# YuanchenBei/ColdRec

Measured on AMD Instinct MI355X. Metric: ranked items/sec (full-catalogue eval), higher is better.
Workload: dtype f32; 1 GPU; configs[3] full-catalogue eval: 1000000-row user table x 10000000 items, d=128, k=20, f32 tables, user block 131072 per step, rated CSR (mean ~50) + 20% cold-item bitmap ('warm' setting), item table row-sharded over 1 GPU(s); items=10000000, dim=128, k=20, parallelism=single GPU

## Files before the change

coldrec_amd/csrc/score_screen.hip:

```cpp
#include <math.h>

#include "score_topk_common.h"

#include <hipcub/device/device_radix_sort.hpp>

namespace crh_score {
namespace {

constexpr int SD = 128;
constexpr int FB_SCRATCH_SLICES = 64;

__device__ __forceinline__ float up_float(double x) {
    if (!(x <= 3.0e38)) return __builtin_inff();
    float f = (float)x;
    if ((double)f < x) f = __uint_as_float(__float_as_uint(f) + 1u);
    return f;
}

__device__ __forceinline__ int scale_exp(const unsigned* stats, int word) {
    const float m = __uint_as_float(stats[word]);
    if (!(m > 0.0f) || !(m <= 3.4e38f)) return 0;
    int E;
    frexpf(m, &E);
    return 15 - E;
}

__device__ __forceinline__ _Float16 to_f16(float x, int e) {
    const float y = ldexpf(x, e);
    _Float16 hv = (_Float16)y;
    if (fabsf((float)hv) < 6.103515625e-05f) hv = (_Float16)0.0f;
    return hv;
}

__device__ __forceinline__ float wave_max(float v) {
#pragma unroll
    for (int o = 32; o >= 1; o >>= 1) v = fmaxf(v, __shfl_xor(v, o));
    return v;
}

constexpr unsigned SCREEN_KEY_NONFINITE = 0x7F80u;
template <bool KEYS>
__global__ __launch_bounds__(256) void screen_maxabs_kernel(const float* __restrict__ tab, const int32_t* __restrict__ rows,
                                                            int64_t n_rows, unsigned* __restrict__ stats, int word,
                                                            uint16_t* __restrict__ keys) {
    const int64_t n4 = n_rows * (SD / 4);
    float m = 0.0f;
    for (int64_t e = (int64_t)blockIdx.x * 256 + threadIdx.x; e < n4; e += (int64_t)gridDim.x * 256) {
        const int64_t r = e / (SD / 4);
        const int64_t row = rows ? (int64_t)rows[r] : r;
        const f32x4 x = *reinterpret_cast<const f32x4*>(tab + row * SD + 4 * (e % (SD / 4)));
#pragma unroll
        for (int c = 0; c < 4; ++c) {
            const float ax = fabsf(x[c]);
            if (ax <= 3.4028235e38f) m = fmaxf(m, ax);
        }
        if constexpr (KEYS) {
            float ss = x[0] * x[0] + x[1] * x[1] + x[2] * x[2] + x[3] * x[3];
#pragma unroll
            for (int o = 16; o >= 1; o >>= 1) ss += __shfl_xor(ss, o);
            if ((threadIdx.x & 31) == 0)
                keys[r] = (uint16_t)(ss <= 3.4028235e38f ? __float_as_uint(ss) >> 16 : SCREEN_KEY_NONFINITE);
        }
    }
    __shared__ float red[4];
    m = wave_max(m);
    if ((threadIdx.x & 63) == 0) red[threadIdx.x >> 6] = m;
    __syncthreads();
    if (threadIdx.x == 0) {
        const float b = fmaxf(fmaxf(red[0], red[1]), fmaxf(red[2], red[3]));
        if (b > 0.0f) atomicMax(stats + word, __float_as_uint(b));
    }
}

__device__ __forceinline__ void row_sums(const f32x4& x0, const f32x4& x1, _Float16 (&hv)[8], int e, double& sxx, double& sdd,
                                         double& shh) {
    const double inv = ldexp(1.0, -e);
    sxx = 0.0; sdd = 0.0; shh = 0.0;
#pragma unroll
    for (int c = 0; c < 8; ++c) {
        const float x = c < 4 ? x0[c & 3] : x1[c & 3];
        hv[c] = to_f16(x, e);
        const double xh = (double)(float)hv[c] * inv;
        const double dx = (double)x - xh;
        sxx += (double)x * (double)x;
        sdd += dx * dx;
        shh += xh * xh;
    }
#pragma unroll
    for (int o = 1; o < 16; o <<= 1) {
        sxx += __shfl_xor(sxx, o);
        sdd += __shfl_xor(sdd, o);
        shh += __shfl_xor(shh, o);
    }
}

__device__ __forceinline__ float up_norm(double s) { return up_float(sqrt(s) * (1.0 + 0x1p-30)); }

constexpr int LIVE_WPB = 256;

__device__ __forceinline__ unsigned live_word(const uint32_t* __restrict__ bitmap, int64_t w, int64_t g0, int64_t g1) {
    const int64_t w0 = g0 >> 5, n_words = ((g1 - 1) >> 5) - w0 + 1;
    if (w >= n_words) return 0u;
    unsigned m = ~bitmap[w0 + w];
    const int64_t lo = (w0 + w) << 5;
    if (lo < g0) m &= ~0u << (int)(g0 - lo);
    if (lo + 32 > g1) m &= ~0u >> (int)(lo + 32 - g1);
    return m;
}

__device__ __forceinline__ unsigned block_excl_sum(unsigned v, unsigned* total) {
    __shared__ unsigned wsum[4];
    const int lane = threadIdx.x & 63, wv = threadIdx.x >> 6;
    unsigned inc = v;
#pragma unroll
    for (int o = 1; o < 64; o <<= 1) {
        const unsigned t = __shfl_up(inc, o);
        if (lane >= o) inc += t;
    }
    if (lane == 63) wsum[wv] = inc;
    __syncthreads();
    unsigned before = 0;
    for (int q = 0; q < wv; ++q) before += wsum[q];
    *total = wsum[0] + wsum[1] + wsum[2] + wsum[3];
    return before + inc - v;
}

__global__ __launch_bounds__(256) void screen_live_count_kernel(const uint32_t* __restrict__ bitmap, int64_t g0, int64_t g1,
                                                                unsigned* __restrict__ blocksum) {
    const unsigned c = __popc(live_word(bitmap, (int64_t)blockIdx.x * LIVE_WPB + threadIdx.x, g0, g1));
    unsigned total;
    block_excl_sum(c, &total);
    if (threadIdx.x == 0) blocksum[blockIdx.x] = total;
}

__global__ __launch_bounds__(256) void screen_live_scan_kernel(unsigned* __restrict__ blocksum, int64_t n_blocks,
                                                               unsigned* __restrict__ n_live) {
    const int64_t per = (n_blocks + 255) / 256;
    const int64_t lo = threadIdx.x * per < n_blocks ? threadIdx.x * per : n_blocks, hi = lo + per < n_blocks ? lo + per : n_blocks;
    unsigned sum = 0;
    for (int64_t q = lo; q < hi; ++q) sum += blocksum[q];
    unsigned total;
    unsigned run = block_excl_sum(sum, &total);
    for (int64_t q = lo; q < hi; ++q) {
        const unsigned c = blocksum[q];
        blocksum[q] = run;
        run += c;
    }
    if (threadIdx.x == 0) *n_live = total;
}

__global__ __launch_bounds__(256) void screen_idmap_kernel(const uint32_t* __restrict__ bitmap, int64_t g0, int64_t g1,
                                                           const unsigned* __restrict__ blocksum, int32_t* __restrict__ idmap) {
    const int64_t w = (int64_t)blockIdx.x * LIVE_WPB + threadIdx.x;
    unsigned m = live_word(bitmap, w, g0, g1);
    unsigned total;
    int64_t pos = (int64_t)blocksum[blockIdx.x] + block_excl_sum(__popc(m), &total);
    const int id0 = (int)(((g0 >> 5) + w) << 5);
    while (m) {
        idmap[pos++] = id0 + __builtin_ctz(m);
        m &= m - 1;
    }
}

__global__ __launch_bounds__(256) void screen_sortkey_kernel(const int32_t* __restrict__ idmap, const uint16_t* __restrict__ rowkeys,
                                                             const unsigned* __restrict__ n_live, int64_t item_base, int64_t n_slots,
                                                             uint16_t* __restrict__ skeys) {
    const int64_t q = (int64_t)blockIdx.x * 256 + threadIdx.x;
    if (q >= n_slots) return;
    skeys[q] = q < (int64_t)*n_live ? (uint16_t)~rowkeys[(int64_t)idmap[q] - item_base] : (uint16_t)0xFFFFu;
}

__global__ __launch_bounds__(256) void screen_mapkeys_kernel(const uint16_t* __restrict__ skeys, int64_t n, int32_t* __restrict__ out) {
    const int64_t q = (int64_t)blockIdx.x * 256 + threadIdx.x;
    if (q < n) out[q] = (int32_t)(uint16_t)~skeys[q];
}

__global__ __launch_bounds__(256) void screen_items_kernel(const float* __restrict__ v, int64_t n_items, const uint32_t* __restrict__ bitmap,
                                                           int64_t item_base, _Float16* __restrict__ packed, unsigned* __restrict__ stats,
                                                           int64_t prefix, const int32_t* __restrict__ idmap) {
    const int e = scale_exp(stats, 0);
    const int64_t TP = prefix >> 5, n_live = idmap ? (int64_t)stats[SCREEN_STAT_LIVE] : 0;
    const int64_t T = idmap ? TP + ((n_live + 31) >> 5) : (n_items + 31) >> 5;
    float mr = 0.0f, mn = 0.0f, mh = 0.0f;
    u32x4* dst = reinterpret_cast<u32x4*>(packed);
    for (int64_t t = blockIdx.x; t < T; t += gridDim.x) {
        for (int p = 0; p < 2; ++p) {
            const int u = threadIdx.x + 256 * p, r = u >> 4, c = u & 15;
            int64_t row = (t << 5) + r;
            bool masked;
            if (idmap != nullptr && t >= TP) {
                const int64_t q = row - prefix;
                masked = q >= n_live;
                row = (int64_t)idmap[masked ? n_live - 1 : q] - item_base;
            } else {
                if (row >= n_items) row = n_items - 1;
                masked = bitmap != nullptr && ((bitmap[(item_base + row) >> 5] >> ((item_base + row) & 31)) & 1u);
            }
            const float* src = v + row * SD + 8 * c;
            const f32x4 x0 = *reinterpret_cast<const f32x4*>(src), x1 = *reinterpret_cast<const f32x4*>(src + 4);
            _Float16 hv[8];
            double sxx, sdd, shh;
            row_sums(x0, x1, hv, e, sxx, sdd, shh);
            u32x4 o = u32x4{0u, 0u, 0u, 0u};
            if (!masked) {
                o = __builtin_bit_cast(u32x4, f16x8{hv[0], hv[1], hv[2], hv[3], hv[4], hv[5], hv[6], hv[7]});
                mr = fmaxf(mr, up_norm(sdd));
                mn = fmaxf(mn, up_norm(sxx));
                mh = fmaxf(mh, up_norm(shh));
                if (sdd != sdd || sxx != sxx) mr = __builtin_inff();
            }
            dst[(t * 8 + (c >> 1)) * 64 + (c & 1) * 32 + r] = o;
        }
    }
    __shared__ float red[3][4];
    mr = wave_max(mr);
    mn = wave_max(mn);
    mh = wave_max(mh);
    if ((threadIdx.x & 63) == 0) {
        red[0][threadIdx.x >> 6] = mr;
        red[1][threadIdx.x >> 6] = mn;
        red[2][threadIdx.x >> 6] = mh;
    }
    __syncthreads();
    if (threadIdx.x < 3) {
        const float b = fmaxf(fmaxf(red[threadIdx.x][0], red[threadIdx.x][1]), fmaxf(red[threadIdx.x][2], red[threadIdx.x][3]));
        if (b > 0.0f) atomicMax(stats + 2 + threadIdx.x, __float_as_uint(b));
    }
}

__global__ __launch_bounds__(256) void screen_users_kernel(const float* __restrict__ uemb, const int32_t* __restrict__ users,
                                                           int64_t n_users, _Float16* __restrict__ uh, float* __restrict__ ustat,
                                                           const unsigned* __restrict__ stats) {
    const int e = scale_exp(stats, 1);
    const int64_t n_units = n_users * 16;
    for (int64_t w = (int64_t)blockIdx.x * 256 + threadIdx.x; w < ((n_units + 255) & ~(int64_t)255); w += (int64_t)gridDim.x * 256) {
        const int64_t j = (w < n_units ? w : n_units - 1) >> 4;
        const int c = (int)(w & 15);
        const int64_t row = users ? (int64_t)users[j] : j;
        const float* src = uemb + row * SD + 8 * c;
        const f32x4 x0 = *reinterpret_cast<const f32x4*>(src), x1 = *reinterpret_cast<const f32x4*>(src + 4);
        _Float16 hv[8];
        double sxx, sdd, shh;
        row_sums(x0, x1, hv, e, sxx, sdd, shh);
        if (w < n_units) {
            reinterpret_cast<u32x4*>(uh)[j * 16 + c] = __builtin_bit_cast(u32x4, f16x8{hv[0], hv[1], hv[2], hv[3], hv[4], hv[5], hv[6], hv[7]});
            if (c == 0) {
                const bool bad = sxx != sxx || sdd != sdd;
                ustat[3 * j + 0] = bad ? __builtin_inff() : up_norm(sxx);
                ustat[3 * j + 1] = bad ? __builtin_inff() : up_norm(shh);
                ustat[3 * j + 2] = bad ? __builtin_inff() : up_norm(sdd);
            }
        }
    }
}

__device__ __forceinline__ float exact_chain(const float* __restrict__ u, const float* __restrict__ v) {
    float s = 0.0f;
#pragma unroll 8
    for (int q = 0; q < SD; q += 4) {
        const f32x4 a = *reinterpret_cast<const f32x4*>(u + q), b = *reinterpret_cast<const f32x4*>(v + q);
        s = __builtin_fmaf(a.x, b.x, s);
        s = __builtin_fmaf(a.y, b.y, s);
        s = __builtin_fmaf(a.z, b.z, s);
        s = __builtin_fmaf(a.w, b.w, s);
    }
    return s;
}

__device__ __forceinline__ bool lane_in_list(const int32_t* __restrict__ col, int64_t lo, int64_t hi, int gi) {
    while (lo < hi) {
        const int64_t mid = lo + ((hi - lo) >> 1);
        const int x = col[mid];
        if (x == gi) return true;
        if (x < gi) lo = mid + 1;
        else hi = mid;
    }
    return false;
}

__global__ __launch_bounds__(256) void screen_certify_kernel(ScreenArgs s) {
    const int lane = threadIdx.x & 63;
    const int64_t slot = (int64_t)blockIdx.x * 4 + (threadIdx.x >> 6);
    if (slot >= s.n_users) return;
    const int KP = s.kp, K = s.k;
    const bool mine = lane < KP;
    int gi = CRH_PAD_IDX;
    float a = CRH_NEG_INF;
    if (mine) {
        gi = s.cand_idx[slot * KP + lane];
        a = s.cand_score[slot * KP + lane];
    }
    const bool real = mine && gi != CRH_PAD_IDX && (int64_t)gi >= s.item_base && (int64_t)gi < s.item_base + s.n_items;
    bool masked = false;
    if (real && s.bitmap) masked = (s.bitmap[gi >> 5] >> (gi & 31)) & 1u;
    if (real && !masked && s.rated_rowptr) masked = lane_in_list(s.rated_col, s.rated_rowptr[slot], s.rated_rowptr[slot + 1], gi);
    const int64_t urow = s.users ? (int64_t)s.users[slot] : slot;
    float sc = CRH_NEG_INF;
    if (real) sc = exact_chain(s.user_emb + urow * SD, s.item_emb + ((int64_t)gi - s.item_base) * SD);
    const bool ok = !mine || (real && !masked && __builtin_isfinite(a) && __builtin_isfinite(sc));
    int rank = 0;
    for (int j = 0; j < KP; ++j) {
        const float sj = __shfl(sc, j);
        const int ij = __shfl(gi, j);
        rank += (j != lane && crh_better(sj, ij, sc, gi)) ? 1 : 0;
    }
    const unsigned long long kth = __ballot(mine && rank == K - 1);
    const float ek = __shfl(sc, kth ? __builtin_ctzll(kth) : 0);
    const float a_last = __shfl(a, KP - 1);
    bool cert = s.mode != 3 && __ballot(!ok) == 0ull && kth != 0ull;
    if (cert) {
        const float* us = s.ustat + 3 * slot;
        const float R = __uint_as_float(s.stats[2]), N = __uint_as_float(s.stats[3]), Nh = __uint_as_float(s.stats[4]);
        const double gd = SD * 0x1p-24 / (1.0 - SD * 0x1p-24), gp = 0x1p-12;
        double B = (double)us[0] * R + (double)us[2] * Nh + gd * (double)us[0] * N + gp * (double)us[1] * Nh + 0x1p-126;
        B *= 1.0 + 0x1p-20;
        const double A = (double)a_last * ldexp(1.0, -(scale_exp(s.stats, 0) + scale_exp(s.stats, 1)));
        double thr = A + B;
        thr += fabs(thr) * 0x1p-50;
        cert = (double)ek > thr && ek > CRH_MASKED_SCORE;
    }
    if (cert) {
        if (mine && rank < K) {
            s.out_score[slot * K + rank] = sc;
            s.out_idx[slot * K + rank] = gi;
        }
    } else if (lane == 0) {
        const unsigned f = atomicAdd(s.stats + 5, 1u);
        s.fail_list[f] = (int32_t)slot;
    }
}

constexpr int64_t FB_WAVES = 2048 * 4;
constexpr int64_t FB_MIN_ITEMS = 1024;
constexpr int FB_FANIN = 64;
constexpr int FB_SLICES_MAX = FB_FANIN * FB_FANIN;
__device__ __forceinline__ int fb_slices(const ScreenArgs& s, int64_t count) {
    if (count <= 0) return 1;
    int64_t S = (FB_WAVES + count - 1) / count;
    const int64_t by_items = (s.n_items + FB_MIN_ITEMS - 1) / FB_MIN_ITEMS;
    const int64_t by_scratch = s.n_users * s.n_slices / count;
    if (S > by_items) S = by_items;
    if (S > by_scratch) S = by_scratch;
    if (S > FB_SLICES_MAX) S = FB_SLICES_MAX;
    return S < 1 ? 1 : (int)S;
}

__global__ __launch_bounds__(256) void screen_fallback_kernel(ScreenArgs s) {
    __shared__ float ush[4][SD];
    __shared__ float lsh[4][32];
    __shared__ int lih[4][32];
    __shared__ int cnth[4];
    const int lane = threadIdx.x & 63, wv = threadIdx.x >> 6;
    const int K = s.k;
    const int64_t count = s.stats[5];
    const int S = fb_slices(s, count);
    const int64_t n_work = count * S;
    float* ls = lsh[wv];
    int* li = lih[wv];
    int* cnt = &cnth[wv];
    for (int64_t w = (int64_t)blockIdx.x * 4 + wv; w < n_work; w += (int64_t)gridDim.x * 4) {
        const int64_t f = w / S;
        const int z = (int)(w % S);
        const int64_t slot = s.fail_list[f];
        const int64_t urow = s.users ? (int64_t)s.users[slot] : slot;
        ush[wv][lane] = s.user_emb[urow * SD + lane];
        ush[wv][lane + 64] = s.user_emb[urow * SD + lane + 64];
        if (lane == 0) *cnt = 0;
        const int64_t lo = s.n_items * z / S, hi = s.n_items * (z + 1) / S;
        float tau = CRH_NEG_INF;
        for (int64_t base = lo; base < hi; base += 64) {
            const int64_t i = base + lane;
            const bool valid = i < hi;
            const int gl = (int)(s.item_base + (valid ? i : lo));
            const bool bm = valid && s.bitmap && ((s.bitmap[gl >> 5] >> (gl & 31)) & 1u);
            float raw = CRH_NEG_INF;
            if (valid) {
                if (bm) {
                    raw = 0.0f;
#pragma unroll 8
                    for (int q = 0; q < SD; ++q) raw = __builtin_fmaf(ush[wv][q], 0.0f, raw);
                } else {
                    raw = exact_chain(ush[wv], s.item_emb + i * SD);
                }
            }
            unsigned long long cand = __ballot(valid && raw > tau);
            const unsigned long long bms = __ballot(bm);
            while (cand) {
                const int L = __builtin_ctzll(cand);
                cand &= cand - 1;
                float sc = __shfl(raw, L);
                const int g = (int)(s.item_base + base + L);
                const int n = __builtin_amdgcn_readfirstlane(*cnt);
                if (wave_list_rejects(ls, li, n, K, sc, g)) continue;
                bool masked = (bms >> L) & 1ull;
                if (!masked && s.rated_rowptr) masked = wave_is_masked(g, slot, s.rated_rowptr, s.rated_col, nullptr, lane);
                if (masked) sc = CRH_MASKED_SCORE;
                wave_list_insert(ls, li, cnt, K, sc, g, lane);
                tau = wave_list_tau(ls, __builtin_amdgcn_readfirstlane(*cnt), K);
            }
        }
        const int n = __builtin_amdgcn_readfirstlane(*cnt);
        const int64_t o = (f * S + z) * K;
        wave_list_store(ls, li, n, K, s.part_score + o, s.part_idx + o, lane);
    }
}

__global__ __launch_bounds__(256) void screen_fallback_merge_kernel(ScreenArgs s, int level) {
    __shared__ float lsh[4][32];
    __shared__ int lih[4][32];
    __shared__ int cnth[4];
    const int lane = threadIdx.x & 63, wv = threadIdx.x >> 6;
    const int K = s.k;
    const int64_t count = s.stats[5];
    const int S = fb_slices(s, count);
    const int last = S <= FB_FANIN ? 0 : 1;
    if (level > last) return;
    const int stride = level == 0 ? 1 : FB_FANIN;
    const int span = stride * FB_FANIN;
    const int G = (S + span - 1) / span;
    float* ls = lsh[wv];
    int* li = lih[wv];
    int* cnt = &cnth[wv];
    for (int64_t w = (int64_t)blockIdx.x * 4 + wv; w < count * G; w += (int64_t)gridDim.x * 4) {
        const int64_t f = w / G;
        const int z0 = (int)(w % G) * span;
        if (lane == 0) *cnt = 0;
        for (int z = z0; z < z0 + span && z < S; z += stride) {
            const int64_t o = (f * S + z) * K;
            const float es = lane < K ? s.part_score[o + lane] : CRH_NEG_INF;
            const int ei = lane < K ? s.part_idx[o + lane] : CRH_PAD_IDX;
            unsigned long long m = __ballot(lane < K && ei != CRH_PAD_IDX);
            while (m) {
                const int L = __builtin_ctzll(m);
                m &= m - 1;
                const float sc = __shfl(es, L);
                const int g = __shfl(ei, L);
                const int n = __builtin_amdgcn_readfirstlane(*cnt);
                if (n >= K && !crh_better(sc, g, ls[K - 1], li[K - 1])) break;
                wave_list_insert(ls, li, cnt, K, sc, g, lane);
            }
        }
        const int n = __builtin_amdgcn_readfirstlane(*cnt);
        if (level == last) {
            const int64_t slot = s.fail_list[f];
            wave_list_store(ls, li, n, K, s.out_score + slot * K, s.out_idx + slot * K, lane);
        } else {
            const int64_t o = (f * S + z0) * K;
            wave_list_store(ls, li, n, K, s.part_score + o, s.part_idx + o, lane);
        }
    }
}

}

int screen_fallback_slices(int64_t n_items) {
    const int64_t s = n_items / 4096;
    return (int)(s < 1 ? 1 : (s > FB_SCRATCH_SLICES ? FB_SCRATCH_SLICES : s));
}

size_t screen_scan_bytes(int64_t n_main) { return (size_t)((n_main + 31) / 32 / LIVE_WPB + 2) * sizeof(unsigned); }

int64_t screen_map_slots(int64_t n_main) { return ((n_main + 31) / 32 + 1) * 32; }

size_t screen_sort_bytes(int64_t n_slots) { return (size_t)n_slots * 8 + ((size_t)1 << 20); }

int launch_screen_map(const uint32_t* bitmap, int64_t item_base, int64_t n_items, int64_t prefix, unsigned* n_live, unsigned* scan,
                      int32_t* idmap, const ScreenOrder* ord, hipStream_t st) {
    const int64_t g0 = item_base + prefix, g1 = item_base + n_items;
    const int64_t n_words = ((g1 - 1) >> 5) - (g0 >> 5) + 1, nb = (n_words + LIVE_WPB - 1) / LIVE_WPB;
    hipLaunchKernelGGL(screen_live_count_kernel, dim3((unsigned)nb), dim3(256), 0, st, bitmap, g0, g1, scan);
    CRH_HIP(hipGetLastError());
    hipLaunchKernelGGL(screen_live_scan_kernel, dim3(1), dim3(256), 0, st, scan, nb, n_live);
    CRH_HIP(hipGetLastError());
    hipLaunchKernelGGL(screen_idmap_kernel, dim3((unsigned)nb), dim3(256), 0, st, bitmap, g0, g1, scan, idmap);
    CRH_HIP(hipGetLastError());
    if (ord == nullptr) return CRH_OK;
    const int64_t n_slots = screen_map_slots(n_items - prefix);
    hipLaunchKernelGGL(screen_sortkey_kernel, dim3((unsigned)((n_slots + 255) / 256)), dim3(256), 0, st, idmap, ord->rowkeys, n_live,
                       item_base, n_slots, ord->skeys_in);
    CRH_HIP(hipGetLastError());
    size_t need = 0;
    CRH_HIP(hipcub::DeviceRadixSort::SortPairs(nullptr, need, ord->skeys_in, ord->skeys_out, idmap, ord->idmap, (int)n_slots, 0, 16, st));
    if (need > ord->sort_tmp_bytes) {
        crh_set_error("screened route: the ordered map's sort asks for %zu bytes of temporary storage, %zu are reserved", need,
                      ord->sort_tmp_bytes);
        return CRH_ERR_WS;
    }
    need = ord->sort_tmp_bytes;
    CRH_HIP(hipcub::DeviceRadixSort::SortPairs(ord->sort_tmp, need, ord->skeys_in, ord->skeys_out, idmap, ord->idmap, (int)n_slots, 0, 16, st));
    return CRH_OK;
}

int launch_screen_prep_items(const ScreenArgs& s, unsigned* stats, _Float16* packed, int64_t prefix, int32_t* idmap, unsigned* scan,
                             const ScreenOrder* ord, hipStream_t st) {
    const int64_t T = (s.n_items + 31) / 32;
    if (ord != nullptr)
        hipLaunchKernelGGL(screen_maxabs_kernel<true>, dim3(2048), dim3(256), 0, st, s.item_emb, nullptr, s.n_items, stats, 0, ord->rowkeys);
    else
        hipLaunchKernelGGL(screen_maxabs_kernel<false>, dim3(2048), dim3(256), 0, st, s.item_emb, nullptr, s.n_items, stats, 0, nullptr);
    CRH_HIP(hipGetLastError());
    if (idmap != nullptr) {
        const int rc = launch_screen_map(s.bitmap, s.item_base, s.n_items, prefix, stats + SCREEN_STAT_LIVE, scan, idmap, ord, st);
        if (rc != CRH_OK) return rc;
        if (ord != nullptr) idmap = ord->idmap;
    }
    hipLaunchKernelGGL(screen_items_kernel, dim3((unsigned)(T < 4096 ? T : 4096)), dim3(256), 0, st, s.item_emb, s.n_items, s.bitmap,
                       s.item_base, packed, stats, prefix, idmap);
    CRH_HIP(hipGetLastError());
    return CRH_OK;
}

int launch_screen_prep_users(const ScreenArgs& s, _Float16* uh, hipStream_t st) {
    hipLaunchKernelGGL(screen_maxabs_kernel<false>, dim3(256), dim3(256), 0, st, s.user_emb, s.users, s.n_users, s.stats, 1, nullptr);
    CRH_HIP(hipGetLastError());
    const int64_t ub = (s.n_users * 16 + 255) / 256;
    hipLaunchKernelGGL(screen_users_kernel, dim3((unsigned)(ub < 2048 ? ub : 2048)), dim3(256), 0, st, s.user_emb, s.users, s.n_users,
                       uh, s.ustat, s.stats);
    CRH_HIP(hipGetLastError());
    return CRH_OK;
}

int screen_map_only(const uint32_t* bitmap, const float* item_emb, int64_t n_items, int64_t item_base, int64_t prefix, int ordered,
                    int32_t* map_out, int32_t* keys_out, int64_t* count, hipStream_t st) {
    auto al = [](size_t x) { return (x + 255) & ~(size_t)255; };
    const int64_t n_main = n_items - prefix, n_slots = screen_map_slots(n_main);
    const size_t o_scan = 256, o_map = o_scan + al(screen_scan_bytes(n_main)), o_rk = o_map + al((size_t)n_slots * 4),
                 o_k0 = o_rk + al((size_t)n_items * 2), o_k1 = o_k0 + al((size_t)n_slots * 2), o_m1 = o_k1 + al((size_t)n_slots * 2),
                 o_tmp = o_m1 + al((size_t)n_slots * 4), total = o_tmp + screen_sort_bytes(n_slots);
    char* buf = nullptr;
    CRH_HIP(hipMalloc(reinterpret_cast<void**>(&buf), total));
    ScreenOrder ord;
    ord.rowkeys = reinterpret_cast<uint16_t*>(buf + o_rk);
    ord.skeys_in = reinterpret_cast<uint16_t*>(buf + o_k0);
    ord.skeys_out = reinterpret_cast<uint16_t*>(buf + o_k1);
    ord.idmap = reinterpret_cast<int32_t*>(buf + o_m1);
    ord.sort_tmp = buf + o_tmp;
    ord.sort_tmp_bytes = screen_sort_bytes(n_slots);
    unsigned* stats = reinterpret_cast<unsigned*>(buf);
    int32_t* idmap = reinterpret_cast<int32_t*>(buf + o_map);
    int rc = CRH_OK;
    unsigned live = 0;
    hipError_t e = hipMemsetAsync(buf, 0, 256, st);
    if (e == hipSuccess) {
        hipLaunchKernelGGL(screen_maxabs_kernel<true>, dim3(2048), dim3(256), 0, st, item_emb, nullptr, n_items, stats, 0, ord.rowkeys);
        e = hipGetLastError();
    }
    if (e == hipSuccess) rc = launch_screen_map(bitmap, item_base, n_items, prefix, stats + SCREEN_STAT_LIVE, reinterpret_cast<unsigned*>(buf + o_scan), idmap, &ord, st);
    if (e == hipSuccess && rc == CRH_OK) {
        hipLaunchKernelGGL(screen_mapkeys_kernel, dim3((unsigned)((n_main + 255) / 256)), dim3(256), 0, st,
                           ordered ? ord.skeys_out : ord.skeys_in, n_main, keys_out);
        e = hipGetLastError();
    }
    if (e == hipSuccess && rc == CRH_OK)
        e = hipMemcpyAsync(map_out, ordered ? ord.idmap : idmap, (size_t)n_main * 4, hipMemcpyDeviceToDevice, st);
    if (e == hipSuccess && rc == CRH_OK) e = hipMemcpyAsync(&live, stats + SCREEN_STAT_LIVE, 4, hipMemcpyDeviceToHost, st);
    if (e == hipSuccess) e = hipStreamSynchronize(st);
    (void)hipFree(buf);
    CRH_HIP(e);
    if (rc == CRH_OK) *count = (int64_t)live;
    return rc;
}

int launch_screen_certify(const ScreenArgs& s, hipStream_t st) {
    hipLaunchKernelGGL(screen_certify_kernel, dim3((unsigned)((s.n_users + 3) / 4)), dim3(256), 0, st, s);
    CRH_HIP(hipGetLastError());
    hipLaunchKernelGGL(screen_fallback_kernel, dim3((unsigned)(FB_WAVES / 4)), dim3(256), 0, st, s);
    CRH_HIP(hipGetLastError());
    for (int level = 0; level < 2; ++level) {
        hipLaunchKernelGGL(screen_fallback_merge_kernel, dim3(512), dim3(256), 0, st, s, level);
        CRH_HIP(hipGetLastError());
    }
    return CRH_OK;
}

}
```

Measured before the change: 6721 billion items/s.

## Batch fallback users per wave and seed fallback threshold from screen candidates

Result: no change. 6761 billion items/s, median of 6 (+0.6%).

```diff
diff --git a/coldrec_amd/csrc/score_screen.hip b/coldrec_amd/csrc/score_screen.hip
--- a/coldrec_amd/csrc/score_screen.hip
+++ b/coldrec_amd/csrc/score_screen.hip
@@ -324,11 +324,32 @@
             s.out_score[slot * K + rank] = sc;
             s.out_idx[slot * K + rank] = gi;
         }
-    } else if (lane == 0) {
-        const unsigned f = atomicAdd(s.stats + 5, 1u);
-        s.fail_list[f] = (int32_t)slot;
-    }
-}
+    } else {
+        const bool good = real && !masked && __builtin_isfinite(sc);
+        const float s2 = good ? sc : CRH_NEG_INF;
+        const int g2 = good ? gi : CRH_PAD_IDX;
+        int r2 = 0;
+        for (int j = 0; j < KP; ++j) {
+            const float sj = __shfl(s2, j);
+            const int ij = __shfl(g2, j);
+            r2 += (j != lane && crh_better(sj, ij, s2, g2)) ? 1 : 0;
+        }
+        const unsigned long long k2 = __ballot(good && r2 == K - 1);
+        float seed = __shfl(s2, k2 ? __builtin_ctzll(k2) : 0);
+        if (k2 == 0ull || !(seed > CRH_MASKED_SCORE)) seed = CRH_NEG_INF;
+        if (lane == 0) {
+            const unsigned f = atomicAdd(s.stats + 5, 1u);
+            s.fail_list[f] = (int32_t)slot;
+            s.ustat[3 * slot] = seed;
+        }
+    }
+}
+
+#ifdef CRH_SCREEN_FALLBACK_PER_USER
+constexpr int FB_GROUP = 1;
+#else
+constexpr int FB_GROUP = 4;
+#endif
 
 constexpr int64_t FB_WAVES = 2048 * 4;
 constexpr int64_t FB_MIN_ITEMS = 1024;
@@ -336,7 +357,8 @@
 constexpr int FB_SLICES_MAX = FB_FANIN * FB_FANIN;
 __device__ __forceinline__ int fb_slices(const ScreenArgs& s, int64_t count) {
     if (count <= 0) return 1;
-    int64_t S = (FB_WAVES + count - 1) / count;
+    const int64_t groups = (count + FB_GROUP - 1) / FB_GROUP;
+    int64_t S = (FB_WAVES + groups - 1) / groups;
     const int64_t by_items = (s.n_items + FB_MIN_ITEMS - 1) / FB_MIN_ITEMS;
     const int64_t by_scratch = s.n_users * s.n_slices / count;
     if (S > by_items) S = by_items;
@@ -345,63 +367,108 @@
     return S < 1 ? 1 : (int)S;
 }
 
+template <int NU>
+__device__ __forceinline__ void exact_chain_group(const float* __restrict__ u, const float* __restrict__ v, float (&sc)[FB_GROUP]) {
+#pragma unroll
+    for (int j = 0; j < NU; ++j) sc[j] = 0.0f;
+#pragma unroll 8
+    for (int q = 0; q < SD; q += 4) {
+        const f32x4 b = *reinterpret_cast<const f32x4*>(v + q);
+#pragma unroll
+        for (int j = 0; j < NU; ++j) {
+            const f32x4 a = *reinterpret_cast<const f32x4*>(u + j * SD + q);
+            sc[j] = __builtin_fmaf(a.x, b.x, sc[j]);
+            sc[j] = __builtin_fmaf(a.y, b.y, sc[j]);
+            sc[j] = __builtin_fmaf(a.z, b.z, sc[j]);
+            sc[j] = __builtin_fmaf(a.w, b.w, sc[j]);
+        }
+    }
+}
+
 __global__ __launch_bounds__(256) void screen_fallback_kernel(ScreenArgs s) {
-    __shared__ float ush[4][SD];
-    __shared__ float lsh[4][32];
-    __shared__ int lih[4][32];
-    __shared__ int cnth[4];
+    __shared__ __attribute__((aligned(16))) float ush[4][FB_GROUP][SD];
+    __shared__ float lsh[4][FB_GROUP][32];
+    __shared__ int lih[4][FB_GROUP][32];
+    __shared__ int cnth[4][FB_GROUP];
     const int lane = threadIdx.x & 63, wv = threadIdx.x >> 6;
     const int K = s.k;
     const int64_t count = s.stats[5];
     const int S = fb_slices(s, count);
-    const int64_t n_work = count * S;
-    float* ls = lsh[wv];
-    int* li = lih[wv];
-    int* cnt = &cnth[wv];
+    const int64_t n_work = (count + FB_GROUP - 1) / FB_GROUP * S;
+    const float* us = &ush[wv][0][0];
     for (int64_t w = (int64_t)blockIdx.x * 4 + wv; w < n_work; w += (int64_t)gridDim.x * 4) {
-        const int64_t f = w / S;
+        const int64_t f0 = w / S * FB_GROUP;
         const int z = (int)(w % S);
-        const int64_t slot = s.fail_list[f];
-        const int64_t urow = s.users ? (int64_t)s.users[slot] : slot;
-        ush[wv][lane] = s.user_emb[urow * SD + lane];
-        ush[wv][lane + 64] = s.user_emb[urow * SD + lane + 64];
-        if (lane == 0) *cnt = 0;
+        const int nu = (int)(count - f0 < FB_GROUP ? count - f0 : FB_GROUP);
+        int64_t slot[FB_GROUP];
+        float tau[FB_GROUP], seed[FB_GROUP];
+#pragma unroll
+        for (int j = 0; j < FB_GROUP; ++j) {
+            slot[j] = s.fail_list[f0 + (j < nu ? j : 0)];
+            const int64_t urow = s.users ? (int64_t)s.users[slot[j]] : slot[j];
+            ush[wv][j][lane] = s.user_emb[urow * SD + lane];
+            ush[wv][j][lane + 64] = s.user_emb[urow * SD + lane + 64];
+            if (lane == 0) cnth[wv][j] = 0;
+            tau[j] = CRH_NEG_INF;
+            seed[j] = FB_GROUP > 1 ? s.ustat[3 * slot[j]] : CRH_NEG_INF;
+        }
         const int64_t lo = s.n_items * z / S, hi = s.n_items * (z + 1) / S;
-        float tau = CRH_NEG_INF;
         for (int64_t base = lo; base < hi; base += 64) {
             const int64_t i = base + lane;
             const bool valid = i < hi;
             const int gl = (int)(s.item_base + (valid ? i : lo));
             const bool bm = valid && s.bitmap && ((s.bitmap[gl >> 5] >> (gl & 31)) & 1u);
-            float raw = CRH_NEG_INF;
+            float raw[FB_GROUP];
+#pragma unroll
+            for (int j = 0; j < FB_GROUP; ++j) raw[j] = CRH_NEG_INF;
             if (valid) {
                 if (bm) {
-                    raw = 0.0f;
+#pragma unroll
+                    for (int j = 0; j < FB_GROUP; ++j) {
+                        if (j < nu) {
+                            raw[j] = 0.0f;
 #pragma unroll 8
-                    for (int q = 0; q < SD; ++q) raw = __builtin_fmaf(ush[wv][q], 0.0f, raw);
+                            for (int q = 0; q < SD; ++q) raw[j] = __builtin_fmaf(us[j * SD + q], 0.0f, raw[j]);
+                        }
+                    }
                 } else {
-                    raw = exact_chain(ush[wv], s.item_emb + i * SD);
+                    const float* v = s.item_emb + i * SD;
+                    if (FB_GROUP == 1 || nu == 1) exact_chain_group<1>(us, v, raw);
+                    else if (nu == 2) exact_chain_group<2 <= FB_GROUP ? 2 : 1>(us, v, raw);
+                    else if (nu == 3) exact_chain_group<3 <= FB_GROUP ? 3 : 1>(us, v, raw);
+                    else exact_chain_group<FB_GROUP>(us, v, raw);
                 }
             }
-            unsigned long long cand = __ballot(valid && raw > tau);
             const unsigned long long bms = __ballot(bm);
-            while (cand) {
-                const int L = __builtin_ctzll(cand);
-                cand &= cand - 1;
-                float sc = __shfl(raw, L);
-                const int g = (int)(s.item_base + base + L);
-                const int n = __builtin_amdgcn_readfirstlane(*cnt);
-                if (wave_list_rejects(ls, li, n, K, sc, g)) continue;
-                bool masked = (bms >> L) & 1ull;
-                if (!masked && s.rated_rowptr) masked = wave_is_masked(g, slot, s.rated_rowptr, s.rated_col, nullptr, lane);
-                if (masked) sc = CRH_MASKED_SCORE;
-                wave_list_insert(ls, li, cnt, K, sc, g, lane);
-                tau = wave_list_tau(ls, __builtin_amdgcn_readfirstlane(*cnt), K);
+#pragma unroll
+            for (int j = 0; j < FB_GROUP; ++j) {
+                if (j >= nu) break;
+                float* ls = lsh[wv][j];
+                int* li = lih[wv][j];
+                int* cnt = &cnth[wv][j];
+                unsigned long long cand = __ballot(valid && raw[j] > tau[j] && raw[j] >= seed[j]);
+                while (cand) {
+                    const int L = __builtin_ctzll(cand);
+                    cand &= cand - 1;
+                    float sc = __shfl(raw[j], L);
+                    const int g = (int)(s.item_base + base + L);
+                    const int n = __builtin_amdgcn_readfirstlane(*cnt);
+                    if (wave_list_rejects(ls, li, n, K, sc, g)) continue;
+                    bool masked = (bms >> L) & 1ull;
+                    if (!masked && s.rated_rowptr) masked = wave_is_masked(g, slot[j], s.rated_rowptr, s.rated_col, nullptr, lane);
+                    if (masked) sc = CRH_MASKED_SCORE;
+                    wave_list_insert(ls, li, cnt, K, sc, g, lane);
+                    tau[j] = wave_list_tau(ls, __builtin_amdgcn_readfirstlane(*cnt), K);
+                }
             }
         }
-        const int n = __builtin_amdgcn_readfirstlane(*cnt);
-        const int64_t o = (f * S + z) * K;
-        wave_list_store(ls, li, n, K, s.part_score + o, s.part_idx + o, lane);
+#pragma unroll
+        for (int j = 0; j < FB_GROUP; ++j) {
+            if (j >= nu) break;
+            const int n = __builtin_amdgcn_readfirstlane(cnth[wv][j]);
+            const int64_t o = ((f0 + j) * S + z) * K;
+            wave_list_store(lsh[wv][j], lih[wv][j], n, K, s.part_score + o, s.part_idx + o, lane);
+        }
     }
 }
 
```
